# briangodwinlim/SIR-GCN

Measured on AMD Instinct MI355X. Metric: edges/sec SIRConv fwd+bwd, d_hidden=256, 1/2/4/8 MI355X, higher is better.
Workload: dtype f32; 1 GPU; cfg4 S2: Chung-Lu power-law V=2000000 E=40000000 alpha=0.8; 1 SIRConv layer d_in=H=d_out=256, agg=sum, LeakyReLU(0.2), f32, feat_dropout=0.0; fwd+bwd incl. projections; graph=S2, V=2000000, E=40000000, hidden=256, agg=sum, parallelism=single GPU

## Files before the change

### sir-gcn_amd/csrc/sirconv_gemm.hip

```cpp
#include <type_traits>
#include <algorithm>

#include "sirconv_internal.h"
#include "sirconv_gemm_util.h"
#include "sirconv_dropout.h"
#include "sirconv_gemm_nt.h"

namespace sir {
namespace {
using namespace gemm;

__device__ inline void kahan_add(float& s, float& c, float x) {
    const float y = x - c;
    const float t = s + y;
    c = (t - s) - y;
    s = t;
}

__device__ inline float gate_dact(float g, float x, int relu, float slope) {
    return g > 0.f ? x : (relu ? 0.f : x * slope);
}
__global__ void __launch_bounds__(256)
k_gate_dact_bits(float* __restrict__ C, int64_t ldc, const uint64_t* __restrict__ mask, int64_t M, int relu, float slope) {
    const int64_t i = (int64_t)blockIdx.x * 256 + threadIdx.x;
// ... 454 lines not shown
                }
            }
            __syncthreads();
#pragma unroll
            for (int i = 0; i < 8; ++i) {
                const int ir = wq + 8 * i, c16 = lq;
                u4v v = *reinterpret_cast<const u4v*>(img + ir * PITCH + c16 * 16);
                const int ml = (ir >> 5) * (TDT * 32) + 32 * b + (ir & 31);
                const int n = p.f0 + 4 * c16;
                const uint32_t off = (n < N) ? (uint32_t)ml * ldc4 + (uint32_t)c16 * 16u : nrec;
                if constexpr (GATE == 2) {
                    const u4v m01 = __builtin_amdgcn_raw_buffer_load_b128(grs, (uint32_t)ml * 32u, 0, 0);
                    const u4v m23 = __builtin_amdgcn_raw_buffer_load_b128(grs, (uint32_t)ml * 32u + 16u, 0, 0);
                    const int sh = c16 & 31;
                    const uint32_t w0 = c16 < 32 ? m01.x : m01.y, w1 = c16 < 32 ? m01.z : m01.w;
                    const uint32_t w2 = c16 < 32 ? m23.x : m23.y, w3 = c16 < 32 ? m23.z : m23.w;
                    const float g0 = ((w0 >> sh) & 1u) ? 1.f : -1.f, g1 = ((w1 >> sh) & 1u) ? 1.f : -1.f;
                    const float g2 = ((w2 >> sh) & 1u) ? 1.f : -1.f, g3 = ((w3 >> sh) & 1u) ? 1.f : -1.f;
                    v.x = __float_as_uint(gate_dact(g0, __uint_as_float(v.x), gate_relu, gate_slope));
                    v.y = __float_as_uint(gate_dact(g1, __uint_as_float(v.y), gate_relu, gate_slope));
                    v.z = __float_as_uint(gate_dact(g2, __uint_as_float(v.z), gate_relu, gate_slope));
                    v.w = __float_as_uint(gate_dact(g3, __uint_as_float(v.w), gate_relu, gate_slope));
                } else if constexpr (GATE == 1) {
                    const u4v gv = __builtin_amdgcn_raw_buffer_load_b128(grs, off, p.f0 * 4, 0);
                    v.x = __float_as_uint(gate_dact(__uint_as_float(gv.x), __uint_as_float(v.x), gate_relu, gate_slope));
                    v.y = __float_as_uint(gate_dact(__uint_as_float(gv.y), __uint_as_float(v.y), gate_relu, gate_slope));
                    v.z = __float_as_uint(gate_dact(__uint_as_float(gv.z), __uint_as_float(v.z), gate_relu, gate_slope));
                    v.w = __float_as_uint(gate_dact(__uint_as_float(gv.w), __uint_as_float(v.w), gate_relu, gate_slope));
                }
                __builtin_amdgcn_raw_buffer_store_b128(v, crs, off, p.f0 * 4, 0);
                __builtin_amdgcn_sched_barrier(0);
                asm volatile("s_nop 1" ::: "memory");
                __builtin_amdgcn_sched_barrier(0);
            }
            __syncthreads();
        }
    };

    TileP cur = tile_p(tb), nxt = tile_p(tb + 1);
    load_a(0, cur, 0);
    load_w(cur, 0);
    store(0, 0, true, false, 0);
    load_a(1, cur, 1);
    load_w(cur, 1);
    load_a(0, cur, 2);
    __syncthreads();
    typedef std::integral_constant<int, 0> I0;
    typedef std::integral_constant<int, 1> I1;
    typedef std::integral_constant<int, 2> I2;
    auto step = [&](int c, int j, const TileP& cu, const TileP& nx, auto P_, auto Z_, auto SK_, auto WN_, auto AN_) {
        constexpr int P = decltype(P_)::value, SK = decltype(SK_)::value;
        constexpr bool Z = decltype(Z_)::value != 0, WN = decltype(WN_)::value != 0, AN = decltype(AN_)::value != 0;
        if constexpr (!Z) rescale(P);
        mfma(P, Z);
        if constexpr (SK == 2) store(0, 0, true, false, 0);
        else store(P ^ 1, P ^ 1, false, SK == 1, j & 1);
        if constexpr (WN) load_w(nx, c + 2 - NCT);
        else load_w(cu, c + 2);
        if constexpr (AN) load_a(P ^ 1, nx, c + 3 - NCT);
        else load_a(P ^ 1, cu, c + 3);
        __syncthreads();
    };
    auto run = [&]() {
        TileP cu = cur, nx = nxt;
        for (int j = 0; tb + j < te; ++j) {
            const TileP nn = tile_p(tb + j + 2);
            step(0, j, cu, nx, I0(), I1(), I0(), I0(), I0());
#pragma unroll
            for (int c = 1; c + 1 <= NCT - 4; c += 2) {
                step(c, j, cu, nx, I1(), I0(), I0(), I0(), I0());
                step(c + 1, j, cu, nx, I0(), I0(), I0(), I0(), I0());
            }
            step(NCT - 3, j, cu, nx, I1(), I0(), I0(), I0(), I1());
            step(NCT - 2, j, cu, nx, I0(), I0(), I1(), I1(), I1());
            step(NCT - 1, j, cu, nx, I1(), I0(), I2(), I1(), I1());
            epilogue(cu, j & 1);
            cu = nx;
            nx = nn;
        }
    };
    run();
}

template <int WM, int WN, int TMT, int TNT>
__global__ void __launch_bounds__(64 * WM * WN)
k_gemm_tn(const float* __restrict__ A, int64_t lda, const float* __restrict__ B, int64_t ldb,
          int64_t R, int Mc, int Nc, float* __restrict__ part, float* __restrict__ csum_part,
          int n_mtiles, int n_ntiles, int64_t rows_per_split) {
    constexpr int NT = 64 * WM * WN;
    constexpr int BM = 32 * TMT * WM, BN = 32 * TNT * WN;
    constexpr int KSPT = 2 * (BM + BN) / NT;
    static_assert(KSPT * NT == 2 * (BM + BN) && (KSPT == 1 || KSPT == 2), "loader mapping");
    constexpr int XR = 16 * KSPT;
    constexpr int A_BYTES = BM * 128, B_BYTES = BN * 128;
    constexpr int STAGE = A_BYTES + B_BYTES + (BM + BN) * 4;
    __shared__ __attribute__((aligned(16))) char lds[2 * STAGE + 16];
    int* const rescaled = reinterpret_cast<int*>(lds + 2 * STAGE);

    const int t = threadIdx.x;
    const int wg = xcd_remap(blockIdx.x, gridDim.x);
    const int tiles = n_mtiles * n_ntiles;
    const int p = wg / tiles, tile = wg % tiles;
    const int m0 = (tile / n_ntiles) * BM, n0 = (tile % n_ntiles) * BN;
    const int64_t v_begin = (int64_t)p * rows_per_split;
    const int64_t v_end = (v_begin + rows_per_split < R) ? v_begin + rows_per_split : R;
    const int nc = (int)((v_end - v_begin + KC - 1) / KC);

    const int slot = KSPT == 1 ? (t >> 1) : t;
    const bool is_a = __builtin_amdgcn_readfirstlane(t >> 6) < BM * (2 / KSPT) / 64;
    const int cl = is_a ? slot : slot - BM, kse = KSPT == 1 ? (t & 1) : 0;
    const bool col_ok = is_a ? (m0 + cl < Mc) : (n0 + cl < Nc);
    const float* xbase = is_a ? A : B;
    const int ldx = (int)(is_a ? lda : ldb);
    const int xoff = 16 * kse * ldx + (is_a ? m0 : n0) + (col_ok ? cl : 0);
    const int img = is_a ? 0 : A_BYTES, rows_img = is_a ? BM : BN, fac_off = is_a ? cl : BM + cl;
    const int hi_off = img + kse * rows_img * 32 + fimg(cl, 0);
    const int lo_delta = 2 * rows_img * 32;
    const int fac_byte = A_BYTES + B_BYTES + fac_off * 4;
    int se_run = SE_INIT;

    const int w = t >> 6, l = t & 63, r = l & 31, h = l >> 5;
    const int m_w = (w / WN) * TMT * 32, n_w = (w % WN) * TNT * 32;

    float4 xv_[2][XR / 4];
    const bool do_cs = csum_part != nullptr && is_a;
    float cs = 0.f, csc = 0.f;
    auto load = [&](int set, int c) {
        float4 (&xv)[XR / 4] = xv_[set];
        const int64_t vc = v_begin + (int64_t)c * KC;
        const float* src = xbase + vc * ldx;
        float x[XR];
        const int64_t nrow = v_end - vc;
        const rsrc_t rs = mk_rsrc(src, nrow <= 0 ? 0u : (uint32_t)((nrow < KC ? nrow : KC) * ldx * 4));
#pragma unroll
        for (int j = 0; j < XR; ++j)
            x[j] = __uint_as_float(__builtin_amdgcn_raw_buffer_load_b32(rs, xoff * 4, j * ldx * 4, 0));
#pragma unroll
        for (int j = 0; j < XR / 4; ++j) xv[j] = make_float4(x[4 * j], x[4 * j + 1], x[4 * j + 2], x[4 * j + 3]);
    };
    auto store = [&](int set, int buf, int chunk, bool first = false) {
        const float4 (&xv)[XR / 4] = xv_[set];
        char* st = lds + buf * STAGE;
        float m = 0.f;
#pragma unroll
        for (int j = 0; j < XR / 4; ++j) m = fmax4_mix(m, xv[j]);
        if (KSPT == 1) m = fmaxf(m, __shfl_xor(m, 1));
        const int se_old = se_run, se = next_se(se_old, bexp(m));
        se_run = se;
        const float s = pow2(se);
#pragma unroll
        for (int q = 0; q < KSPT; ++q) {
            h8 hv[2], lv[2];
            split8_mix(xv[4 * q + 0], xv[4 * q + 1], s, hv[0], lv[0]);
            split8_mix(xv[4 * q + 2], xv[4 * q + 3], s, hv[1], lv[1]);
            char* hd = st + hi_off + q * rows_img * 32;
            *reinterpret_cast<h8*>(hd) = hv[0];
            *reinterpret_cast<h8*>(hd + 512) = hv[1];
            *reinterpret_cast<h8*>(hd + lo_delta) = lv[0];
            *reinterpret_cast<h8*>(hd + lo_delta + 512) = lv[1];
        }
        if (kse == 0) *reinterpret_cast<float*>(st + fac_byte) = first ? 1.f : pow2(se - se_old);
        if (do_cs) {
            float t = 0.f;
#pragma unroll
            for (int j = 0; j < XR / 4; ++j) { t += xv[j].x; t += xv[j].y; t += xv[j].z; t += xv[j].w; }
            kahan_add(cs, csc, t);
        }
        if (!first && se != se_old) rescaled[buf] = chunk;
    };

    f16v acc[TMT][TNT];
#pragma unroll
    for (int a = 0; a < TMT; ++a)
#pragma unroll
        for (int b = 0; b < TNT; ++b)
#pragma unroll
            for (int i = 0; i < 16; ++i) acc[a][b][i] = 0.f;

    auto compute = [&](int c) {
        const int buf = c & 1;
        const char* st = lds + buf * STAGE;
        if (rescaled[buf] == c) {
            const float* fac = reinterpret_cast<const float*>(st + A_BYTES + B_BYTES);
#pragma unroll
            for (int a = 0; a < TMT; ++a) {
                float fa[16];
#pragma unroll
                for (int g = 0; g < 4; ++g) {
                    const float4 f4 = *reinterpret_cast<const float4*>(fac + m_w + 32 * a + 8 * g + 4 * h);
                    fa[4 * g] = f4.x; fa[4 * g + 1] = f4.y; fa[4 * g + 2] = f4.z; fa[4 * g + 3] = f4.w;
                }
#pragma unroll
                for (int b = 0; b < TNT; ++b) {
                    const float fb = fac[BM + n_w + 32 * b + r];
#pragma unroll
                    for (int i = 0; i < 16; ++i) acc[a][b][i] *= fa[i] * fb;
                }
            }
        }
#pragma unroll
        for (int ks = 0; ks < 2; ++ks) {
            __builtin_amdgcn_sched_barrier(0);
            h8 af[TMT][2], bf[TNT][2];
#pragma unroll
            for (int pt = 0; pt < 2; ++pt) {
#pragma unroll
                for (int a = 0; a < TMT; ++a)
                    af[a][pt] = *reinterpret_cast<const h8*>(st + (pt * 2 + ks) * BM * 32 + fimg(m_w + 32 * a + r, h));
#pragma unroll
                for (int b = 0; b < TNT; ++b)
                    bf[b][pt] = *reinterpret_cast<const h8*>(st + A_BYTES + (pt * 2 + ks) * BN * 32 + fimg(n_w + 32 * b + r, h));
            }
#pragma unroll
            for (int a = 0; a < TMT; ++a)
#pragma unroll
                for (int b = 0; b < TNT; ++b)
                    acc[a][b] = __builtin_amdgcn_mfma_f32_32x32x16_f16(af[a][0], bf[b][0], acc[a][b], 0, 0, 0);
#pragma unroll
            for (int a = 0; a < TMT; ++a)
#pragma unroll
                for (int b = 0; b < TNT; ++b)
                    acc[a][b] = __builtin_amdgcn_mfma_f32_32x32x16_f16(af[a][0], bf[b][1], acc[a][b], 0, 0, 0);
#pragma unroll
            for (int a = 0; a < TMT; ++a)
#pragma unroll
                for (int b = 0; b < TNT; ++b)
                    acc[a][b] = __builtin_amdgcn_mfma_f32_32x32x16_f16(af[a][1], bf[b][0], acc[a][b], 0, 0, 0);
        }
    };

    if (t < 2) rescaled[t] = -1;
    if (nc > 0) {
        load(0, 0);
        load(1, 1);
        store(0, 0, 0, true);
    }
    __syncthreads();
    auto step = [&](int c, int set) {
        load(set, c + 2);
        compute(c);
        if (c + 1 < nc) store(set ^ 1, (c + 1) & 1, c + 1);
        __syncthreads();
    };
    int c = 0;
    for (; c + 2 <= nc; c += 2) {
        step(c, 0);
        step(c + 1, 1);
    }
    if (c < nc) step(c, 0);

    float* sc = reinterpret_cast<float*>(lds);
    if (kse == 0) sc[fac_off] = pow2(-se_run);
    __syncthreads();
    float* out = part + (int64_t)p * Mc * Nc;
#pragma unroll
    for (int b = 0; b < TNT; ++b) {
        const int nl = n_w + 32 * b + r;
        const int n = n0 + nl;
        const float ib = sc[BM + nl];
#pragma unroll
        for (int a = 0; a < TMT; ++a) {
#pragma unroll
            for (int i = 0; i < 16; ++i) {
                const int ml = m_w + 32 * a + (i & 3) + 8 * (i >> 2) + 4 * h;
                const int m = m0 + ml;
                if (m < Mc && n < Nc) out[(int64_t)m * Nc + n] = acc[a][b][i] * sc[ml] * ib;
            }
        }
    }
    if (do_cs && tile % n_ntiles == 0) {
        const float other = KSPT == 1 ? __shfl_xor(cs, 1) : 0.f;
        if (kse == 0 && col_ok) csum_part[(int64_t)p * Mc + m0 + cl] = KSPT == 1 ? cs + other : cs;
    }
}

__global__ void __launch_bounds__(256)
k_gemm_reduce(const float* __restrict__ part, int P, int64_t count, int Nc, float* __restrict__ C, int64_t ldc) {
    const int64_t i = (int64_t)blockIdx.x * 256 + threadIdx.x;
    if (i >= count) return;
    float s = 0.f;
    int q = 0;
    for (; q + 16 <= P; q += 16) {
        float v[16];
#pragma unroll
        for (int j = 0; j < 16; ++j) v[j] = part[(int64_t)(q + j) * count + i];
#pragma unroll
        for (int j = 0; j < 16; ++j) s += v[j];
    }
    for (; q < P; ++q) s += part[(int64_t)q * count + i];
    C[(i / Nc) * ldc + i % Nc] = s;
}

constexpr int S_FT = 2;

template <bool KFULL>
__global__ void __launch_bounds__(256)
k_gemm_nt_s(const float* __restrict__ A, int64_t lda, int64_t M, int K, const u4v* __restrict__ Wp, int Npad, int Kc,
            const float* __restrict__ inv_t, const float* __restrict__ bias, int N, float* __restrict__ C, int64_t ldc,
            int nfg, int64_t n_waves, Drop drop) {
    drop = drop_resolve(drop);
    const int l = threadIdx.x & 63, r = l & 31, h = l >> 5;
    const int64_t w = (int64_t)blockIdx.x * 4 + (threadIdx.x >> 6);
    if (w >= n_waves) return;
    const int64_t d0 = (w / nfg) * 32;
    const int f0 = (int)(w % nfg) * S_FT;
    const int rows = (M - d0 < 32) ? (int)(M - d0) : 32;
    const rsrc_t ars = mk_rsrc(A + d0 * lda, (uint32_t)(rows * lda * 4));
    const rsrc_t wrs = mk_rsrc(Wp, (uint32_t)((int64_t)Kc * 4 * Npad * 32));
    const int aoff = (r * (int)lda + 8 * h) * 4;
    const int woff = 16 * l;
    float4 av[2][4];
    u4v wv[2][S_FT][2][2];
    auto load = [&](int set, int c) {
#pragma unroll
        for (int i = 0; i < 4; ++i) {
            const u4v u = __builtin_amdgcn_raw_buffer_load_b128(ars, aoff + ((i >> 1) * 16 + (i & 1) * 4) * 4, c * KC * 4, 0);
            av[set][i] = make_float4(__uint_as_float(u.x), __uint_as_float(u.y), __uint_as_float(u.z), __uint_as_float(u.w));
        }
#pragma unroll
        for (int a = 0; a < S_FT; ++a)
#pragma unroll
            for (int pt = 0; pt < 2; ++pt)
#pragma unroll
                for (int ks = 0; ks < 2; ++ks)
                    wv[set][a][pt][ks] = __builtin_amdgcn_raw_buffer_load_b128(
                        wrs, woff, ((c * 2 + pt) * 2 + ks) * Npad * 32 + (f0 + a) * 1024, 0);
    };
    f16v acc[S_FT];
#pragma unroll
    for (int a = 0; a < S_FT; ++a)
#pragma unroll
        for (int i = 0; i < 16; ++i) acc[a][i] = 0.f;
// ... 469 lines not shown
    float pv[16];
    tile.result(pv, h);
    wait_vm<0>();
    __syncthreads();
    float* red = lds;
    float* cred = lds + G::RED;
    const int tile_id = w0 + W0 * w1;
    if (wk > 0) {
#pragma unroll
        for (int i = 0; i < 16; ++i) red[(((wk - 1) * W0 * W1 + tile_id) * 16 + i) * 64 + l] = pv[i];
    }
    if (do_cs) cred[(wk * G::L0 + w0 * 32 + j) * 2 + h] = tile.cs;
    __syncthreads();
    if (wk == 0) {
#pragma unroll
        for (int q = 1; q < WK; ++q) {
#pragma unroll
            for (int i = 0; i < 16; ++i) pv[i] += red[(((q - 1) * W0 * W1 + tile_id) * 16 + i) * 64 + l];
        }
        const int64_t r1 = a1 + 32 * w1 + j;
        if constexpr (EPI == 0) {
            if (r1 < n1lines) {
#pragma unroll
                for (int g = 0; g < 4; ++g) {
                    const int64_t n = a0 + 32 * w0 + 8 * g + 4 * h;
                    if (n < n0lines) {
                        float4 o = make_float4(pv[4 * g] + bb[g].x, pv[4 * g + 1] + bb[g].y, pv[4 * g + 2] + bb[g].z,
                                               pv[4 * g + 3] + bb[g].w);
                        if (drop.on()) drop4(drop, r1, (int)n, o);
                        *reinterpret_cast<float4*>(C + r1 * ldc + n) = o;
                    }
                }
            }
        } else {
            float* out = C + p * n0lines * n1lines;
            if (r1 < n1lines) {
#pragma unroll
                for (int i = 0; i < 16; ++i) {
                    const int64_t m = a0 + 32 * w0 + (i & 3) + 8 * (i >> 2) + 4 * h;
                    if (m < n0lines) out[m * n1lines + r1] = pv[i];
                }
            }
        }
    }
    SIR_LT_TRACE_AT(20, __builtin_amdgcn_s_memtime());
    SIR_LT_TRACE_AT(21, __builtin_amdgcn_s_memrealtime());
    if (do_cs && t < G::L0 && a0 + t < n0lines) {
        float sum = 0.f;
#pragma unroll
        for (int q = 0; q < WK; ++q) sum += cred[(q * G::L0 + t) * 2] + cred[(q * G::L0 + t) * 2 + 1];
        csum_part[p * n0lines + a0 + t] = sum;
    }
}

}

#ifndef SIR_SMALL_ROWS
#define SIR_SMALL_ROWS 16384
#endif
static int64_t gemm_small_rows() {
    const char* e = getenv("SIR_GEMM_SMALL_ROWS");
    return (e != nullptr && e[0] != 0) ? atoll(e) : (int64_t)SIR_SMALL_ROWS;
}

#ifndef SIR_TN_S_ROWS
#define SIR_TN_S_ROWS 512
#endif
#ifndef SIR_LT_NT
#define SIR_LT_NT -1
#endif
#ifndef SIR_LT_TN
#define SIR_LT_TN 2
#endif
static int lt_env(const char* name, int dflt) {
    const char* e = getenv(name);
    return (e != nullptr && e[0] != 0) ? atoi(e) : dflt;
}
#ifndef SIR_NT_2B
#define SIR_NT_2B -1
#endif
static bool nt_2b_auto(int K, int N) {
    return (K == 256 && (N == 256 || N == 512)) || (K == 512 && N == 256);
}
#ifndef SIR_LT_BLOCKS
#define SIR_LT_BLOCKS 512
#endif
static bool aligned16(const void* p, int64_t ld) { return ((uintptr_t)p & 15u) == 0 && ld % 4 == 0; }
static int gemm_tn_splits_lt(int64_t R, int64_t tiles, int KS, int64_t* rps) {
    int64_t P = (SIR_LT_BLOCKS + tiles - 1) / tiles;
    const int64_t pmax = (R + KS - 1) / KS;
    if (P > pmax) P = pmax;
    if (P > 32) P = 32;
    if (P < 1) P = 1;
    int64_t r = (R + P - 1) / P;
    r = (r + KS - 1) / KS * KS;
    *rps = r > 0 ? r : KS;
    P = (R + *rps - 1) / *rps;
    return (int)(P < 1 ? 1 : P);
}

static int gemm_tn_splits_s(int64_t R, int64_t, int64_t) {
    int64_t P = (R + SIR_TN_S_ROWS - 1) / SIR_TN_S_ROWS;
    if (P > 16) P = 16;
    if (P < 1) P = 1;
    return (int)P;
}

static hipError_t run_gemm_nt_s(const float* A, int64_t lda, int64_t M, int K, const void* packed, int N,
                                const float* bias, float* C, int64_t ldc, hipStream_t st, const Drop& drop) {
    const int np = (int)gemm_pack_npad(N), kc = (K + KC - 1) / KC;
    const u4v* wp = static_cast<const u4v*>(packed);
    const float* inv = reinterpret_cast<const float*>(static_cast<const char*>(packed) + (int64_t)kc * 4 * np * 32);
    const int nfg = (N + 32 * S_FT - 1) / (32 * S_FT);
    const int64_t waves = (M + 31) / 32 * nfg;
    const unsigned blocks = (unsigned)((waves + 3) / 4);
    if (K % KC == 0)
        hipLaunchKernelGGL(k_gemm_nt_s<true>, dim3(blocks), dim3(256), 0, st, A, lda, M, K, wp, np, kc, inv, bias, N, C,
                           ldc, nfg, waves, drop);
    else
        hipLaunchKernelGGL(k_gemm_nt_s<false>, dim3(blocks), dim3(256), 0, st, A, lda, M, K, wp, np, kc, inv, bias, N, C,
                           ldc, nfg, waves, drop);
    return hipGetLastError();
}

#ifndef SIR_LT_NS
#define SIR_LT_NS 3
#endif
struct NtW {
    const float* W;
    int64_t ldw;
    const float* W2;
    int64_t ldw2, split, bias_cols;
};
template <bool TRANS, int W0, int W1, int WK>
static void launch_nt_lt(const float* A, int64_t lda, int64_t M, int K, const NtW& w, int N, const float* bias,
                         float* C, int64_t ldc, hipStream_t st, const Drop& drop) {
    using G = Lt<!TRANS, true, W0, W1, WK, SIR_LT_NS>;
    const int nt0 = (N + G::L0 - 1) / G::L0;
    const int64_t nt1 = (M + G::L1 - 1) / G::L1;
    hipLaunchKernelGGL((k_gemm_lt<!TRANS, true, W0, W1, WK, SIR_LT_NS, 0>), dim3((unsigned)(nt0 * nt1)), dim3(G::NT), 0, st,
                       w.W, w.ldw, A, lda, (int64_t)N, M, (int64_t)K, nt0, (int)nt1, (int64_t)K, bias, C, ldc, nullptr,
                       drop, w.W2, w.ldw2, w.split, w.bias_cols);
}

static int nt_lt_auto(int64_t M, int N) {
    const int64_t ncu = device_cu_count();
    if ((int64_t)((N + 31) / 32) * ((M + 63) / 64) <= ncu) return 7;
    if ((int64_t)((N + 63) / 64) * ((M + 63) / 64) <= ncu) return 8;
    return 3;
}

hipError_t run_gemm_nt_direct(const float* A, int64_t lda, int64_t M, int K, const float* W, int64_t ldw, int trans,
                              int N, const float* bias, float* C, int64_t ldc, hipStream_t st, const Drop& drop,
                              const float* W2, int64_t ldw2, int64_t split, int64_t bias_cols) {
    if (M == 0 || N == 0) return hipSuccess;
    int lt = lt_env("SIR_LT_NT", SIR_LT_NT);
    if (lt < 0) lt = nt_lt_auto(M, N);
    const NtW w{W, ldw, W2, ldw2, W2 != nullptr ? split : INT64_MAX, bias_cols};
    if (lt > 0 && K % 4 == 0 && N % 4 == 0 && aligned16(A, lda) && aligned16(W, ldw) && ((uintptr_t)bias & 15u) == 0
        && (W2 == nullptr || aligned16(W2, ldw2)) && 128 * lda < ((int64_t)1 << 29)
        && (trans ? (int64_t)K * ldw : 128 * ldw) < ((int64_t)1 << 29)
        && (M + 31) / 32 * ((N + 31) / 32) < ((int64_t)1 << 31)) {
        switch (lt * 2 + (trans ? 1 : 0)) {
        case 2: launch_nt_lt<false, 2, 2, 1>(A, lda, M, K, w, N, bias, C, ldc, st, drop); break;
        case 3: launch_nt_lt<true, 2, 2, 1>(A, lda, M, K, w, N, bias, C, ldc, st, drop); break;
        case 4: launch_nt_lt<false, 1, 2, 2>(A, lda, M, K, w, N, bias, C, ldc, st, drop); break;
// ... 125 lines not shown

hipError_t run_gemm_reduce(const float* part, int P, int64_t count, int Nc, float* C, int64_t ldc, hipStream_t st) {
    if (count > 0)
        hipLaunchKernelGGL(k_gemm_reduce, dim3((unsigned)((count + 255) / 256)), dim3(256), 0, st, part, P, count, Nc, C,
                           ldc);
    return hipGetLastError();
}

#ifndef SIR_TN_MINROWS
#define SIR_TN_MINROWS 1024
#endif
int gemm_tn_splits(int64_t R, int64_t Mc, int64_t Nc) {
    const int64_t tiles = ((Mc + 255) / 256) * ((Nc + 255) / 256);
    int64_t P = (256 + tiles - 1) / tiles;
    const int64_t pmax = (R + SIR_TN_MINROWS - 1) / SIR_TN_MINROWS;
    if (P > pmax) P = pmax;
    if (P < 1) P = 1;
    return (int)P;
}

int64_t gemm_tn_workspace(int64_t R, int64_t Mc, int64_t Nc) {
    int64_t P = gemm_tn_splits(R, Mc, Nc);
    if (R < gemm_small_rows()) {
        const int64_t ps = gemm_tn_splits_s(R, Mc, Nc);
        if (ps > P) P = ps;
        if (P < 32) P = 32;
    }
    return P * (Mc * Nc + Mc) * 4;
}

static int lt_tn_w0(int lt) { return (lt == 1 || lt == 5) ? 2 : 1; }
static int lt_tn_w1(int lt) { return lt == 3 ? 1 : 2; }
static int lt_tn_ks(int lt) { return 32 * (lt == 1 ? 1 : (lt == 2 || lt == 5) ? 2 : 4); }
static int64_t lt_tn_tiles(int lt, int Mc, int Nc) {
    const int a = 32 * lt_tn_w0(lt), b = 32 * lt_tn_w1(lt);
    return (int64_t)((Mc + a - 1) / a) * ((Nc + b - 1) / b);
}
template <int W0, int W1, int WK>
static void launch_tn_lt(const float* A, int64_t lda, const float* B, int64_t ldb, int64_t R, int Mc, int Nc,
                         float* part, bool colsum, hipStream_t st) {
    using G = Lt<false, false, W0, W1, WK, SIR_LT_NS>;
    const int nt0 = (Mc + G::L0 - 1) / G::L0, nt1 = (Nc + G::L1 - 1) / G::L1;
    const int64_t tiles = (int64_t)nt0 * nt1;
    int64_t rl = 0;
    const int Pl = gemm_tn_splits_lt(R, tiles, G::KS, &rl);
    float* cp = colsum ? part + (int64_t)Pl * Mc * Nc : nullptr;
    hipLaunchKernelGGL((k_gemm_lt<false, false, W0, W1, WK, SIR_LT_NS, 1>), dim3((unsigned)(Pl * tiles)), dim3(G::NT), 0,
                       st, A, lda, B, ldb, (int64_t)Mc, (int64_t)Nc, R, nt0, nt1, rl, nullptr, part, (int64_t)0, cp,
                       Drop{});
}

hipError_t run_gemm_tn(const float* A, int64_t lda, const float* B, int64_t ldb, int64_t R, int Mc, int Nc,
                       float* C, int64_t ldc, float* colsum, void* workspace, hipStream_t st) {
    if (Mc == 0 || Nc == 0) return hipSuccess;
    const bool small = R < gemm_small_rows();
    const int P = small ? gemm_tn_splits_s(R, Mc, Nc) : gemm_tn_splits(R, Mc, Nc);
    const int64_t rps = (R + P - 1) / P;
    const int nmt = (Mc + 255) / 256, nnt = (Nc + 255) / 256;
    float* part = static_cast<float*>(workspace);
    float* cpart = colsum != nullptr ? part + (int64_t)P * Mc * Nc : nullptr;
    const int lt = lt_env("SIR_LT_TN", SIR_LT_TN);
    if (small && lt > 0 && lt <= 5 && aligned16(A, lda) && aligned16(B, ldb) && (Mc + 31) / 32 * ((Nc + 31) / 32) < (1 << 24)) {
        switch (lt) {
        case 1: launch_tn_lt<2, 2, 1>(A, lda, B, ldb, R, Mc, Nc, part, colsum != nullptr, st); break;
        case 2: launch_tn_lt<1, 2, 2>(A, lda, B, ldb, R, Mc, Nc, part, colsum != nullptr, st); break;
        case 3: launch_tn_lt<1, 1, 4>(A, lda, B, ldb, R, Mc, Nc, part, colsum != nullptr, st); break;
        case 4: launch_tn_lt<1, 2, 4>(A, lda, B, ldb, R, Mc, Nc, part, colsum != nullptr, st); break;
        default: launch_tn_lt<2, 2, 2>(A, lda, B, ldb, R, Mc, Nc, part, colsum != nullptr, st); break;
        }
        const int64_t tiles = lt_tn_tiles(lt, Mc, Nc);
        int64_t rl = 0;
        const int Pl = gemm_tn_splits_lt(R, tiles, lt_tn_ks(lt), &rl);
        float* cp = colsum != nullptr ? part + (int64_t)Pl * Mc * Nc : nullptr;
        const int64_t count = (int64_t)Mc * Nc;
        const int64_t nbm = (count + 255) / 256, nbc = colsum != nullptr ? (Mc + 255) / 256 : 0;
        hipLaunchKernelGGL(k_gemm_reduce2, dim3((unsigned)(nbm + nbc)), dim3(256), 0, st, part, Pl, count, Nc, C, ldc,
                           cp, Mc, colsum, nbm);
        return hipGetLastError();
    }
    if (small) {
        const int smt = (Mc + 31) / 32, snt = (Nc + 31) / 32;
        hipLaunchKernelGGL(k_gemm_tn_s, dim3((unsigned)((int64_t)P * smt * snt)), dim3(256), 0, st, A, lda, B, ldb, R,
                           Mc, Nc, part, cpart, smt, snt, rps);
    } else
    hipLaunchKernelGGL((k_gemm_tn<2, 4, 4, 2>), dim3((unsigned)(P * nmt * nnt)), dim3(512), 0, st,
                       A, lda, B, ldb, R, Mc, Nc, part, cpart, nmt, nnt, rps);
    const int64_t count = (int64_t)Mc * Nc;
    const int64_t nbm = (count + 255) / 256, nbc = colsum != nullptr ? (Mc + 255) / 256 : 0;
    hipLaunchKernelGGL(k_gemm_reduce2, dim3((unsigned)(nbm + nbc)), dim3(256), 0, st, part, P, count, Nc, C, ldc, cpart,
                       Mc, colsum, nbm);
    return hipGetLastError();
}

}
```

### sir-gcn_amd/csrc/sirconv_gemm16.hip

```cpp
#include "sirconv.h"
#include "sirconv_internal.h"
#include "sirconv_gemm_util.h"
#include "sirconv_dropout.h"

#include <type_traits>

namespace sir {
namespace {
using namespace gemm;

typedef _Float16 h8 __attribute__((ext_vector_type(8)));
typedef __bf16 b8 __attribute__((ext_vector_type(8)));
typedef float f16v __attribute__((ext_vector_type(16)));
typedef unsigned int u4v __attribute__((ext_vector_type(4)));

constexpr int KC16 = 32;
constexpr int NSET = 3;

template <bool BF>
__device__ inline f16v mfma16(u4v a, u4v b, f16v c) {
    if constexpr (BF)
        return __builtin_amdgcn_mfma_f32_32x32x16_bf16(__builtin_bit_cast(b8, a), __builtin_bit_cast(b8, b), c, 0, 0, 0);
    else
        return __builtin_amdgcn_mfma_f32_32x32x16_f16(__builtin_bit_cast(h8, a), __builtin_bit_cast(h8, b), c, 0, 0, 0);
}

template <bool BF, bool C32>
__device__ inline float rnd16(float x) {
    if constexpr (C32) return x;
    else if constexpr (BF) return (float)(__bf16)x;
    else return (float)(_Float16)x;
}

template <bool BF>
__device__ inline float widen(uint32_t bits16) {
    if constexpr (BF)
        return __uint_as_float(bits16 << 16);
    else
        return (float)__builtin_bit_cast(_Float16, (unsigned short)bits16);
}

template <bool BF, int BM = 256, int BN = 256, int WN = 4, int TMT = 4, int TNT = 2>
__global__ void __launch_bounds__(BM + BN)
k_gemm_tn16(const unsigned short* __restrict__ A, int64_t lda, const unsigned short* __restrict__ B, int64_t ldb,
            int64_t R, int Mc, int Nc, float* __restrict__ part, float* __restrict__ csum_part, int n_mtiles,
            int n_ntiles, int64_t rows_per_split) {
    constexpr int SLOTS = BM / 2 + BN / 2;
    constexpr int PLANE_A = BM * 32, PLANE_B = BN * 32;
    constexpr int A_BYTES = 2 * PLANE_A, B_BYTES = 2 * PLANE_B;
    constexpr int STAGE = A_BYTES + B_BYTES;
    static_assert((SLOTS & (SLOTS - 1)) == 0 && (BM / 2) % 64 == 0, "slot layout");
    static_assert((BM / (TMT * 32)) * (BN / (TNT * 32)) == (BM + BN) / 64 && BN / (TNT * 32) == WN, "wave tiling");
    __shared__ __attribute__((aligned(16))) char lds[2 * STAGE];

    const int t = threadIdx.x;
    const int wg = xcd_remap(blockIdx.x, gridDim.x);
    const int tiles = n_mtiles * n_ntiles;
    const int p = wg / tiles, tile = wg % tiles;
    const int m0 = (tile / n_ntiles) * BM, n0 = (tile % n_ntiles) * BN;
    const int64_t v_begin = (int64_t)p * rows_per_split;
    const int64_t v_end = (v_begin + rows_per_split < R) ? v_begin + rows_per_split : R;
    const int nc = v_end > v_begin ? (int)((v_end - v_begin + KC16 - 1) / KC16) : 0;

    const int slot = t & (SLOTS - 1), kse = t / SLOTS;
    const bool is_a = (__builtin_amdgcn_readfirstlane(t >> 6) % (SLOTS / 64)) < (BM / 2) / 64;
    const int pr = is_a ? slot : slot - BM / 2;
    const int c0 = 2 * pr;
    const bool col_ok = is_a ? (m0 + c0 < Mc) : (n0 + c0 < Nc);
    const unsigned short* xbase = is_a ? A : B;
    const int64_t ldx = is_a ? lda : ldb;
    const int voff = ((is_a ? m0 : n0) + (col_ok ? c0 : 0)) * 2 + kse * 16 * (int)ldx * 2;
    const int img = (is_a ? 0 : A_BYTES) + kse * (is_a ? PLANE_A : PLANE_B);

    const int w = t >> 6, l = t & 63, r = l & 31, h = l >> 5;
    const int m_w = (w / WN) * TMT * 32, n_w = (w % WN) * TNT * 32;

    const int rstride = (int)ldx * 2;
    uint32_t xs[NSET][16];
    auto load = [&](int set, int c) {
        const int64_t vc = v_begin + (int64_t)c * KC16;
        const int64_t nrow = v_end - vc;
        const rsrc_t rs = mk_rsrc(xbase + vc * ldx, nrow <= 0 ? 0u : (uint32_t)((nrow < KC16 ? nrow : KC16) * ldx * 2));
        int so = 0;
#pragma unroll
        for (int j = 0; j < 16; ++j) {
            xs[set][j] = __builtin_amdgcn_raw_buffer_load_b32(rs, voff, so, 0);
            so += rstride;
            asm volatile("" : "+s"(so));
        }
    };
    float cs0 = 0.f, cs1 = 0.f;
    const bool do_cs = csum_part != nullptr && is_a;
    auto store = [&](int set, int buf) {
        char* st = lds + buf * STAGE + img;
        u4v lo0, lo1, hi0, hi1;
        uint32_t* q[4] = {(uint32_t*)&lo0, (uint32_t*)&lo1, (uint32_t*)&hi0, (uint32_t*)&hi1};
#pragma unroll
        for (int i = 0; i < 4; ++i) {
            q[0][i] = __builtin_amdgcn_perm(xs[set][2 * i + 1], xs[set][2 * i], 0x05040100u);
            q[1][i] = __builtin_amdgcn_perm(xs[set][2 * i + 9], xs[set][2 * i + 8], 0x05040100u);
            q[2][i] = __builtin_amdgcn_perm(xs[set][2 * i + 1], xs[set][2 * i], 0x07060302u);
            q[3][i] = __builtin_amdgcn_perm(xs[set][2 * i + 9], xs[set][2 * i + 8], 0x07060302u);
        }
        *reinterpret_cast<u4v*>(st + fimg(c0, 0)) = lo0;
        *reinterpret_cast<u4v*>(st + fimg(c0, 1)) = lo1;
        *reinterpret_cast<u4v*>(st + fimg(c0 + 1, 0)) = hi0;
        *reinterpret_cast<u4v*>(st + fimg(c0 + 1, 1)) = hi1;
        if (do_cs) {
#pragma unroll
            for (int j = 0; j < 16; ++j) {
                cs0 += widen<BF>(xs[set][j] & 0xffffu);
                cs1 += widen<BF>(xs[set][j] >> 16);
            }
        }
    };

    f16v acc[TMT][TNT];
#pragma unroll
    for (int a = 0; a < TMT; ++a)
#pragma unroll
        for (int b = 0; b < TNT; ++b)
#pragma unroll
            for (int i = 0; i < 16; ++i) acc[a][b][i] = 0.f;

    auto mfma = [&](int buf) {
        const char* st = lds + buf * STAGE;
#pragma unroll
        for (int ks = 0; ks < 2; ++ks) {
            u4v af[TMT], bf[TNT];
#pragma unroll
            for (int a = 0; a < TMT; ++a)
                af[a] = *reinterpret_cast<const u4v*>(st + ks * PLANE_A + fimg(m_w + 32 * a + r, h));
#pragma unroll
            for (int b = 0; b < TNT; ++b)
                bf[b] = *reinterpret_cast<const u4v*>(st + A_BYTES + ks * PLANE_B + fimg(n_w + 32 * b + r, h));
#pragma unroll
            for (int a = 0; a < TMT; ++a)
#pragma unroll
                for (int b = 0; b < TNT; ++b) acc[a][b] = mfma16<BF>(af[a], bf[b], acc[a][b]);
        }
    };

    auto step_full = [&](int c, int s) {
        load(s, c + 3);
        mfma(c & 1);
        store((s + 1) % NSET, (c + 1) & 1);
        __syncthreads();
    };
    auto step_tail = [&](int c, int s) {
        mfma(c & 1);
        if (c + 1 < nc) store((s + 1) % NSET, (c + 1) & 1);
        __syncthreads();
    };
    if (nc > 0) {
        load(0, 0);
        load(1, 1);
        load(2, 2);
        store(0, 0);
        __syncthreads();
        int c = 0;
        for (; c + 3 < nc; c += 3) {
            step_full(c, 0);
            step_full(c + 1, 1);
            step_full(c + 2, 2);
        }
        step_tail(c, 0);
        if (c + 1 < nc) step_tail(c + 1, 1);
        if (c + 2 < nc) step_tail(c + 2, 2);
    }

    float* out = part + (int64_t)p * Mc * Nc;
#pragma unroll
    for (int b = 0; b < TNT; ++b) {
        const int n = n0 + n_w + 32 * b + r;
#pragma unroll
        for (int a = 0; a < TMT; ++a) {
#pragma unroll
            for (int i = 0; i < 16; ++i) {
                const int m = m0 + m_w + 32 * a + (i & 3) + 8 * (i >> 2) + 4 * h;
                if (m < Mc && n < Nc) out[(int64_t)m * Nc + n] = acc[a][b][i];
            }
        }
    }
    if (csum_part != nullptr && tile % n_ntiles == 0) {
        float* cl = reinterpret_cast<float*>(lds);
        __syncthreads();
        if (is_a && kse == 1) { cl[c0] = cs0; cl[c0 + 1] = cs1; }
        __syncthreads();
        if (is_a && kse == 0) {
            if (m0 + c0 < Mc) csum_part[(int64_t)p * Mc + m0 + c0] = cs0 + cl[c0];
            if (m0 + c0 + 1 < Mc) csum_part[(int64_t)p * Mc + m0 + c0 + 1] = cs1 + cl[c0 + 1];
        }
    }
}


template <int I, int N_, typename F>
__device__ __forceinline__ void static_for(F&& f) {
    if constexpr (I < N_) {
        f(std::integral_constant<int, I>());
        static_for<I + 1, N_>(f);
    }
}

__device__ inline uint32_t pack2(float a, float b, bool bf) {
    if (bf) return (uint32_t)__builtin_bit_cast(unsigned short, (__bf16)a) |
                   ((uint32_t)__builtin_bit_cast(unsigned short, (__bf16)b) << 16);
    return (uint32_t)__builtin_bit_cast(unsigned short, (_Float16)a) |
           ((uint32_t)__builtin_bit_cast(unsigned short, (_Float16)b) << 16);
}

template <bool BF, bool A32, bool C32, int KC, int NC, int NS, int BFT = 256>
__global__ void __launch_bounds__(512)
k_gemm_nt16(const void* __restrict__ A, int64_t lda, int64_t M, const u4v* __restrict__ Wp, int Npad,
            const float* __restrict__ bias, int N, void* __restrict__ C, int64_t ldc, unsigned short* __restrict__ Acopy,
            int64_t ldac, int n_ftiles, int n_tiles, int tiles_per_block, Drop drop) {
    drop = drop_resolve(drop);
    constexpr int BD = 256, TFT = 2, WF = BFT / (TFT * 32), WD = 8 / WF, TDT = BD / (WD * 32);
    constexpr int KS = KC / 16;
    constexpr int PLANE = 256 * 32;
    constexpr int PLANE_W = BFT * 32;
    constexpr int STAGE = KS * (PLANE + PLANE_W);
    constexpr int EA = A32 ? 4 : 2;
    constexpr int AV = (KC / 2) * EA / 16;
    constexpr int WV = KS * PLANE_W / (16 * 512);
    constexpr int EC = C32 ? 4 : 2;
    static_assert(KC == 32 || KC == 64, "chunk");
    static_assert(BFT == 256 || BFT == 128, "feature tile");
    static_assert(WV >= 1, "weight loader");
    static_assert(NS >= 2 && NS <= NC && NC % NS == 0, "register sets: a tile's chunks map to sets the same way");
    constexpr int IMG_ROWS = 32 * WD;
    constexpr int EPITCH = BFT * EC + 16;
    constexpr int EPI_BYTES = IMG_ROWS * EPITCH;
    __shared__ __attribute__((aligned(16))) char lds[2 * STAGE + 512 * 4 + EPI_BYTES];
    float* const bias_l = reinterpret_cast<float*>(lds + 2 * STAGE);
    char* const epi = lds + 2 * STAGE + 512 * 4;

// ... 101 lines not shown
#pragma unroll
                for (int g = 0; g < 4; ++g) {
                    const int nl = f_wq + 32 * a + 8 * g + 4 * hq;
                    const float4 bb = *reinterpret_cast<const float4*>(bias_l + p.f0 + nl);
                    float o0 = acc[a][b][4 * g + 0] + bb.x, o1 = acc[a][b][4 * g + 1] + bb.y;
                    float o2 = acc[a][b][4 * g + 2] + bb.z, o3 = acc[a][b][4 * g + 3] + bb.w;
                    if (drop.on()) {
                        const uint32_t rh = drop_row_hash(drop, p.d0 + (wq / WF) * (TDT * 32) + 32 * b + rq);
                        const int cc = drop.col0 + p.f0 + nl;
                        o0 = drop_keep(drop, rh, cc + 0) ? rnd16<BF, C32>(o0) * drop.scale : 0.f;
                        o1 = drop_keep(drop, rh, cc + 1) ? rnd16<BF, C32>(o1) * drop.scale : 0.f;
                        o2 = drop_keep(drop, rh, cc + 2) ? rnd16<BF, C32>(o2) * drop.scale : 0.f;
                        o3 = drop_keep(drop, rh, cc + 3) ? rnd16<BF, C32>(o3) * drop.scale : 0.f;
                    }
                    char* d = wrow + (32 * a + 8 * g) * EC;
                    if constexpr (C32) {
                        *reinterpret_cast<float4*>(d) = make_float4(o0, o1, o2, o3);
                    } else {
                        typedef unsigned int u2v __attribute__((ext_vector_type(2)));
                        u2v ov;
                        ov.x = pack2(o0, o1, BF);
                        ov.y = pack2(o2, o3, BF);
                        *reinterpret_cast<u2v*>(d) = ov;
                    }
                }
            }
            __syncthreads();
            constexpr int PR = BFT * EC / 16;
#pragma unroll
            for (int i = 0; i < IMG_ROWS * PR / 512; ++i) {
                const int q = tq + 512 * i;
                const int ir = q / PR, c16 = q % PR;
                const u4v v = *reinterpret_cast<const u4v*>(epi + ir * EPITCH + c16 * 16);
                const int ml = (ir >> 5) * (TDT * 32) + 32 * b + (ir & 31);
                const int n = p.f0 + c16 * (16 / EC);
                const uint32_t off = (n < N) ? (uint32_t)ml * ldcb + (uint32_t)c16 * 16u : nrec;
                __builtin_amdgcn_raw_buffer_store_b128(v, crs, off, p.f0 * EC, 0);
                __builtin_amdgcn_sched_barrier(0);
                asm volatile("s_nop 1" ::: "memory");
                __builtin_amdgcn_sched_barrier(0);
            }
            __syncthreads();
        }
    };

    TileP cu = tile_p(tb), nx = tile_p(tb + 1);
    static_for<0, NS>([&](auto I_) { load(decltype(I_)::value, cu, decltype(I_)::value); });
    store(0, 0, cu, 0);
    __syncthreads();
    for (int j = 0; tb + j < te; ++j) {
        const TileP nn = tile_p(tb + j + 2);
        static_for<0, NC>([&](auto C_) {
            constexpr int c = decltype(C_)::value;
            constexpr int s = c % NS;
            if constexpr (c + NS < NC) load(s, cu, c + NS);
            else load(s, nx, c + NS - NC);
            mfma(c & 1, c == 0);
            if constexpr (c == NC - 1) epilogue(cu);
            if constexpr (c + 1 < NC) store((c + 1) % NS, (c + 1) & 1, cu, c + 1);
            else store(0, 0, nx, 0);
            __syncthreads();
        });
        cu = nx;
        nx = nn;
    }
}

__global__ void __launch_bounds__(64)
k_pack16(const float* __restrict__ W, int64_t ldw, int N, int K, int trans, int bf, int Npad, unsigned short* __restrict__ out) {
    const int n = blockIdx.x;
    for (int k = threadIdx.x; k < K; k += 64) {
        const float x = (n < N) ? (trans ? W[(int64_t)k * ldw + n] : W[(int64_t)n * ldw + k]) : 0.f;
        const unsigned short b = bf ? __builtin_bit_cast(unsigned short, (__bf16)x) : __builtin_bit_cast(unsigned short, (_Float16)x);
        const int P = k >> 4, j = k & 15;
        out[((int64_t)P * Npad * 32 + fimg(n, j >> 3)) / 2 + (j & 7)] = b;
    }
}

}

#ifndef SIR_TN16_NARROW
#define SIR_TN16_NARROW 1
#endif
static bool tn16_narrow(int Mc, int Nc) {
    const char* e = getenv("SIR_TN16_NARROW");
    const int on = (e != nullptr && e[0] != 0) ? atoi(e) : SIR_TN16_NARROW;
    return on && (Mc <= 128 || Nc <= 128);
}

hipError_t run_gemm_tn16(const void* A, int64_t lda, const void* B, int64_t ldb, int64_t R, int Mc, int Nc, int dtype,
                         float* C, int64_t ldc, float* colsum, void* workspace, hipStream_t st) {
    if (Mc == 0 || Nc == 0) return hipSuccess;
    const int P = gemm_tn_splits(R, Mc, Nc);
    const int64_t rps = (R + P - 1) / P;
    const int nmt = (Mc + 255) / 256, nnt = (Nc + 255) / 256;
    float* part = static_cast<float*>(workspace);
    float* cpart = colsum != nullptr ? part + (int64_t)P * Mc * Nc : nullptr;
    const auto* a = static_cast<const unsigned short*>(A);
    const auto* b = static_cast<const unsigned short*>(B);
    if (tn16_narrow(Mc, Nc)) {
        const int nm = (Mc + 127) / 128, nn = (Nc + 127) / 128;
        const dim3 grid((unsigned)(P * nm * nn));
        if (dtype == SIR_DTYPE_BF16)
            hipLaunchKernelGGL((k_gemm_tn16<true, 128, 128, 2, 2, 2>), grid, dim3(256), 0, st, a, lda, b, ldb, R, Mc, Nc,
                               part, cpart, nm, nn, rps);
        else
            hipLaunchKernelGGL((k_gemm_tn16<false, 128, 128, 2, 2, 2>), grid, dim3(256), 0, st, a, lda, b, ldb, R, Mc, Nc,
                               part, cpart, nm, nn, rps);
    } else {
        const dim3 grid((unsigned)(P * nmt * nnt));
        if (dtype == SIR_DTYPE_BF16)
            hipLaunchKernelGGL(k_gemm_tn16<true>, grid, dim3(512), 0, st, a, lda, b, ldb, R, Mc, Nc, part, cpart, nmt, nnt,
                               rps);
        else
            hipLaunchKernelGGL(k_gemm_tn16<false>, grid, dim3(512), 0, st, a, lda, b, ldb, R, Mc, Nc, part, cpart, nmt, nnt,
                               rps);
    }
    hipError_t e = hipGetLastError();
    if (e != hipSuccess) return e;
    e = run_gemm_reduce(part, P, (int64_t)Mc * Nc, Nc, C, ldc, st);
    if (e != hipSuccess || colsum == nullptr) return e;
    return run_gemm_reduce(cpart, P, (int64_t)Mc, Mc, colsum, 0, st);
}


namespace {
template <int DT>
__global__ void __launch_bounds__(256)
k_dropout_apply(void* __restrict__ X, int64_t ldx, int64_t M, int N, Drop drop) {
    drop = drop_resolve(drop);
    const int64_t m = blockIdx.y;
    const uint32_t rh = drop_row_hash(drop, m);
    for (int n = blockIdx.x * 256 + threadIdx.x; n < N; n += gridDim.x * 256) {
        const bool k = drop_keep(drop, rh, drop.col0 + n);
        if constexpr (DT == SIR_DTYPE_F32) {
            float* p = static_cast<float*>(X) + m * ldx + n;
            *p = k ? *p * drop.scale : 0.f;
        } else if constexpr (DT == SIR_DTYPE_BF16) {
            __bf16* p = static_cast<__bf16*>(X) + m * ldx + n;
            *p = k ? (__bf16)((float)*p * drop.scale) : (__bf16)0.f;
        } else {
            _Float16* p = static_cast<_Float16*>(X) + m * ldx + n;
            *p = k ? (_Float16)((float)*p * drop.scale) : (_Float16)0.f;
        }
    }
}
}

hipError_t run_dropout_apply(void* X, int64_t ldx, int64_t M, int N, int dtype, const Drop& drop, hipStream_t st) {
    if (M == 0 || N == 0 || !drop.on()) return hipSuccess;
    if (M > 2147483647) return hipErrorInvalidValue;
    const dim3 grid((unsigned)((N + 255) / 256 < 4 ? (N + 255) / 256 : 4), (unsigned)M);
    if (dtype == SIR_DTYPE_F32) hipLaunchKernelGGL(k_dropout_apply<SIR_DTYPE_F32>, grid, dim3(256), 0, st, X, ldx, M, N, drop);
    else if (dtype == SIR_DTYPE_BF16) hipLaunchKernelGGL(k_dropout_apply<SIR_DTYPE_BF16>, grid, dim3(256), 0, st, X, ldx, M, N, drop);
    else hipLaunchKernelGGL(k_dropout_apply<SIR_DTYPE_F16>, grid, dim3(256), 0, st, X, ldx, M, N, drop);
    return hipGetLastError();
}

int64_t gemm_pack16_bytes(int64_t N, int64_t K) { return (N + 255) / 256 * 256 * K * 2; }

hipError_t run_gemm_pack16(const float* W, int64_t ldw, int N, int K, int trans, int dtype, void* packed, hipStream_t st) {
    const int np = (N + 255) / 256 * 256;
    hipLaunchKernelGGL(k_pack16, dim3(np), dim3(64), 0, st, W, ldw, N, K, trans, dtype == SIR_DTYPE_BF16 ? 1 : 0, np,
                       static_cast<unsigned short*>(packed));
    return hipGetLastError();
}

#ifndef SIR_NT16_KC
#define SIR_NT16_KC 32
#endif
#ifndef SIR_NT16_NS
#define SIR_NT16_NS 2
#endif
#ifndef SIR_NT16_NS32
#define SIR_NT16_NS32 2
#endif

#ifndef SIR_NT16_NARROW
#define SIR_NT16_NARROW 1
#endif
template <bool BF, bool A32, bool C32, int BFT>
static hipError_t launch_nt16_w(const void* A, int64_t lda, int64_t M, int K, const void* packed, int N, const float* bias,
                                void* C, int64_t ldc, unsigned short* Acopy, int64_t ldac, hipStream_t st, const Drop& drop) {
    const int np = (N + 255) / 256 * 256, nft = (N + BFT - 1) / BFT;
    const int64_t ntiles = (M + 255) / 256 * nft;
    const int ncu = device_cu_count();
    const int tpb = (int)((ntiles + ncu - 1) / ncu);
    const int nblk = (int)((ntiles + tpb - 1) / tpb);
    const auto* wp = static_cast<const u4v*>(packed);
    constexpr int KC = (SIR_NT16_KC == 64 && !A32) ? 64 : 32;
    constexpr int NS = A32 ? SIR_NT16_NS32 : SIR_NT16_NS;
    const int nc = K / KC;
#define SIR_NT16_L(NCV, NSV)                                                                                   \
    hipLaunchKernelGGL((k_gemm_nt16<BF, A32, C32, KC, NCV, NSV, BFT>), dim3((unsigned)nblk), dim3(512), 0, st, A, lda, \
                       M, wp, np, bias, N, C, ldc, Acopy, ldac, nft, (int)ntiles, tpb, drop)
    if (nc == 256 / KC) SIR_NT16_L(256 / KC, (NS <= 256 / KC ? NS : 256 / KC));
// ... 39 lines not shown
```

Baseline: 1.982 billion edges/s.

## Stagger B-loader waves in TN weight-gradient GEMMs to spread LDS stores

Adds a STAG template variant to the f32 and 16-bit TN GEMM kernels. In it, the waves that load B store the next chunk to LDS before issuing the next global load and computing, while the A-loader waves keep the original order. The goal is to desynchronise the global-load and LDS-store phases across waves within a workgroup, so memory traffic and MFMA work overlap better. By default it is enabled only for Nc=256 with Mc=256 or 512. The B waves prefetch one extra chunk ahead, which adds register pressure and makes the pipeline more complex.

```diff
diff --git a/sir-gcn_amd/csrc/sirconv_gemm.hip b/sir-gcn_amd/csrc/sirconv_gemm.hip
--- a/sir-gcn_amd/csrc/sirconv_gemm.hip
+++ b/sir-gcn_amd/csrc/sirconv_gemm.hip
@@ -560,7 +560,7 @@
     run();
 }
 
-template <int WM, int WN, int TMT, int TNT>
+template <int WM, int WN, int TMT, int TNT, bool STAG = false>
 __global__ void __launch_bounds__(64 * WM * WN)
 k_gemm_tn(const float* __restrict__ A, int64_t lda, const float* __restrict__ B, int64_t ldb,
           int64_t R, int Mc, int Nc, float* __restrict__ part, float* __restrict__ csum_part,
@@ -603,7 +603,7 @@
     float4 xv_[2][XR / 4];
     const bool do_cs = csum_part != nullptr && is_a;
     float cs = 0.f, csc = 0.f;
-    auto load = [&](int set, int c) {
+    auto load = [&](int set, int c) __attribute__((always_inline)) {
         float4 (&xv)[XR / 4] = xv_[set];
         const int64_t vc = v_begin + (int64_t)c * KC;
         const float* src = xbase + vc * ldx;
@@ -616,7 +616,7 @@
 #pragma unroll
         for (int j = 0; j < XR / 4; ++j) xv[j] = make_float4(x[4 * j], x[4 * j + 1], x[4 * j + 2], x[4 * j + 3]);
     };
-    auto store = [&](int set, int buf, int chunk, bool first = false) {
+    auto store = [&](int set, int buf, int chunk, bool first = false) __attribute__((always_inline)) {
         const float4 (&xv)[XR / 4] = xv_[set];
         char* st = lds + buf * STAGE;
         float m = 0.f;
@@ -655,7 +655,7 @@
 #pragma unroll
             for (int i = 0; i < 16; ++i) acc[a][b][i] = 0.f;
 
-    auto compute = [&](int c) {
+    auto compute = [&](int c) __attribute__((always_inline)) {
         const int buf = c & 1;
         const char* st = lds + buf * STAGE;
         if (rescaled[buf] == c) {
@@ -708,24 +708,44 @@
     };
 
     if (t < 2) rescaled[t] = -1;
-    if (nc > 0) {
-        load(0, 0);
-        load(1, 1);
-        store(0, 0, 0, true);
-    }
-    __syncthreads();
-    auto step = [&](int c, int set) {
-        load(set, c + 2);
-        compute(c);
-        if (c + 1 < nc) store(set ^ 1, (c + 1) & 1, c + 1);
+    static_assert(!STAG || BM * (2 / KSPT) / 64 == WM * WN / 2, "the late half is the B loaders");
+    const bool late = STAG && !is_a;
+    auto run = [&](auto step) {
+        int c = 0;
+        for (; c + 2 <= nc; c += 2) {
+            step(c, 0);
+            step(c + 1, 1);
+        }
+        if (c < nc) step(c, 0);
+    };
+    if (late) {
+        if (nc > 0) {
+            load(0, 0);
+            load(1, 1);
+            store(0, 0, 0, true);
+            load(0, 2);
+        }
         __syncthreads();
-    };
-    int c = 0;
-    for (; c + 2 <= nc; c += 2) {
-        step(c, 0);
-        step(c + 1, 1);
-    }
-    if (c < nc) step(c, 0);
+        run([&](int c, int set) __attribute__((always_inline)) {
+            if (c + 1 < nc) store(set ^ 1, (c + 1) & 1, c + 1);
+            load(set ^ 1, c + 3);
+            compute(c);
+            __syncthreads();
+        });
+    } else {
+        if (nc > 0) {
+            load(0, 0);
+            load(1, 1);
+            store(0, 0, 0, true);
+        }
+        __syncthreads();
+        run([&](int c, int set) __attribute__((always_inline)) {
+            load(set, c + 2);
+            compute(c);
+            if (c + 1 < nc) store(set ^ 1, (c + 1) & 1, c + 1);
+            __syncthreads();
+        });
+    }
 
     float* sc = reinterpret_cast<float*>(lds);
     if (kse == 0) sc[fac_off] = pow2(-se_run);
@@ -1361,6 +1381,10 @@
 static bool nt_2b_auto(int K, int N) {
     return (K == 256 && (N == 256 || N == 512)) || (K == 512 && N == 256);
 }
+#ifndef SIR_TN_STAG
+#define SIR_TN_STAG -1
+#endif
+static bool tn_stag_auto(int Mc, int Nc) { return Nc == 256 && (Mc == 256 || Mc == 512); }
 #ifndef SIR_LT_BLOCKS
 #define SIR_LT_BLOCKS 512
 #endif
@@ -1652,9 +1676,15 @@
         const int smt = (Mc + 31) / 32, snt = (Nc + 31) / 32;
         hipLaunchKernelGGL(k_gemm_tn_s, dim3((unsigned)((int64_t)P * smt * snt)), dim3(256), 0, st, A, lda, B, ldb, R,
                            Mc, Nc, part, cpart, smt, snt, rps);
-    } else
-    hipLaunchKernelGGL((k_gemm_tn<2, 4, 4, 2>), dim3((unsigned)(P * nmt * nnt)), dim3(512), 0, st,
-                       A, lda, B, ldb, R, Mc, Nc, part, cpart, nmt, nnt, rps);
+    } else {
+        const int stag = lt_env("SIR_TN_STAG", SIR_TN_STAG);
+        if (stag < 0 ? tn_stag_auto(Mc, Nc) : stag != 0)
+            hipLaunchKernelGGL((k_gemm_tn<2, 4, 4, 2, true>), dim3((unsigned)(P * nmt * nnt)), dim3(512), 0, st,
+                               A, lda, B, ldb, R, Mc, Nc, part, cpart, nmt, nnt, rps);
+        else
+            hipLaunchKernelGGL((k_gemm_tn<2, 4, 4, 2, false>), dim3((unsigned)(P * nmt * nnt)), dim3(512), 0, st,
+                               A, lda, B, ldb, R, Mc, Nc, part, cpart, nmt, nnt, rps);
+    }
     const int64_t count = (int64_t)Mc * Nc;
     const int64_t nbm = (count + 255) / 256, nbc = colsum != nullptr ? (Mc + 255) / 256 : 0;
     hipLaunchKernelGGL(k_gemm_reduce2, dim3((unsigned)(nbm + nbc)), dim3(256), 0, st, part, P, count, Nc, C, ldc, cpart,
diff --git a/sir-gcn_amd/csrc/sirconv_gemm16.hip b/sir-gcn_amd/csrc/sirconv_gemm16.hip
--- a/sir-gcn_amd/csrc/sirconv_gemm16.hip
+++ b/sir-gcn_amd/csrc/sirconv_gemm16.hip
@@ -40,7 +40,7 @@
         return (float)__builtin_bit_cast(_Float16, (unsigned short)bits16);
 }
 
-template <bool BF, int BM = 256, int BN = 256, int WN = 4, int TMT = 4, int TNT = 2>
+template <bool BF, int BM = 256, int BN = 256, int WN = 4, int TMT = 4, int TNT = 2, bool STAG = false>
 __global__ void __launch_bounds__(BM + BN)
 k_gemm_tn16(const unsigned short* __restrict__ A, int64_t lda, const unsigned short* __restrict__ B, int64_t ldb,
             int64_t R, int Mc, int Nc, float* __restrict__ part, float* __restrict__ csum_part, int n_mtiles,
@@ -77,7 +77,7 @@
 
     const int rstride = (int)ldx * 2;
     uint32_t xs[NSET][16];
-    auto load = [&](int set, int c) {
+    auto load = [&](int set, int c) __attribute__((always_inline)) {
         const int64_t vc = v_begin + (int64_t)c * KC16;
         const int64_t nrow = v_end - vc;
         const rsrc_t rs = mk_rsrc(xbase + vc * ldx, nrow <= 0 ? 0u : (uint32_t)((nrow < KC16 ? nrow : KC16) * ldx * 2));
@@ -91,7 +91,7 @@
     };
     float cs0 = 0.f, cs1 = 0.f;
     const bool do_cs = csum_part != nullptr && is_a;
-    auto store = [&](int set, int buf) {
+    auto store = [&](int set, int buf) __attribute__((always_inline)) {
         char* st = lds + buf * STAGE + img;
         u4v lo0, lo1, hi0, hi1;
         uint32_t* q[4] = {(uint32_t*)&lo0, (uint32_t*)&lo1, (uint32_t*)&hi0, (uint32_t*)&hi1};
@@ -123,7 +123,7 @@
 #pragma unroll
             for (int i = 0; i < 16; ++i) acc[a][b][i] = 0.f;
 
-    auto mfma = [&](int buf) {
+    auto mfma = [&](int buf) __attribute__((always_inline)) {
         const char* st = lds + buf * STAGE;
 #pragma unroll
         for (int ks = 0; ks < 2; ++ks) {
@@ -141,18 +141,46 @@
         }
     };
 
-    auto step_full = [&](int c, int s) {
-        load(s, c + 3);
-        mfma(c & 1);
-        store((s + 1) % NSET, (c + 1) & 1);
+    const bool late = STAG && __builtin_amdgcn_readfirstlane(t >> 6) >= (BM + BN) / 128;
+    if (nc > 0 && late) {
+        load(0, 0);
+        load(1, 1);
+        load(2, 2);
+        store(0, 0);
+        load(0, 3);
         __syncthreads();
-    };
-    auto step_tail = [&](int c, int s) {
-        mfma(c & 1);
-        if (c + 1 < nc) store((s + 1) % NSET, (c + 1) & 1);
-        __syncthreads();
-    };
-    if (nc > 0) {
+        auto step_full = [&](int c, int s) __attribute__((always_inline)) {
+            store((s + 1) % NSET, (c + 1) & 1);
+            load((s + 1) % NSET, c + 4);
+            mfma(c & 1);
+            __syncthreads();
+        };
+        auto step_tail = [&](int c, int s) __attribute__((always_inline)) {
+            if (c + 1 < nc) store((s + 1) % NSET, (c + 1) & 1);
+            mfma(c & 1);
+            __syncthreads();
+        };
+        int c = 0;
+        for (; c + 3 < nc; c += 3) {
+            step_full(c, 0);
+            step_full(c + 1, 1);
+            step_full(c + 2, 2);
+        }
+        step_tail(c, 0);
+        if (c + 1 < nc) step_tail(c + 1, 1);
+        if (c + 2 < nc) step_tail(c + 2, 2);
+    } else if (nc > 0) {
+        auto step_full = [&](int c, int s) __attribute__((always_inline)) {
+            load(s, c + 3);
+            mfma(c & 1);
+            store((s + 1) % NSET, (c + 1) & 1);
+            __syncthreads();
+        };
+        auto step_tail = [&](int c, int s) __attribute__((always_inline)) {
+            mfma(c & 1);
+            if (c + 1 < nc) store((s + 1) % NSET, (c + 1) & 1);
+            __syncthreads();
+        };
         load(0, 0);
         load(1, 1);
         load(2, 2);
@@ -420,6 +448,14 @@
 #ifndef SIR_TN16_NARROW
 #define SIR_TN16_NARROW 1
 #endif
+#ifndef SIR_TN16_STAG
+#define SIR_TN16_STAG -1
+#endif
+static bool tn16_stag(int Mc, int Nc) {
+    const char* e = getenv("SIR_TN16_STAG");
+    const int v = (e != nullptr && e[0] != 0) ? atoi(e) : SIR_TN16_STAG;
+    return v < 0 ? (Nc == 256 && (Mc == 256 || Mc == 512)) : v != 0;
+}
 static bool tn16_narrow(int Mc, int Nc) {
     const char* e = getenv("SIR_TN16_NARROW");
     const int on = (e != nullptr && e[0] != 0) ? atoi(e) : SIR_TN16_NARROW;
@@ -447,9 +483,16 @@
                                part, cpart, nm, nn, rps);
     } else {
         const dim3 grid((unsigned)(P * nmt * nnt));
-        if (dtype == SIR_DTYPE_BF16)
+        const bool stag = tn16_stag(Mc, Nc);
+        if (dtype == SIR_DTYPE_BF16 && stag)
+            hipLaunchKernelGGL((k_gemm_tn16<true, 256, 256, 4, 4, 2, true>), grid, dim3(512), 0, st, a, lda, b, ldb, R, Mc, Nc,
+                               part, cpart, nmt, nnt, rps);
+        else if (dtype == SIR_DTYPE_BF16)
             hipLaunchKernelGGL(k_gemm_tn16<true>, grid, dim3(512), 0, st, a, lda, b, ldb, R, Mc, Nc, part, cpart, nmt, nnt,
                                rps);
+        else if (stag)
+            hipLaunchKernelGGL((k_gemm_tn16<false, 256, 256, 4, 4, 2, true>), grid, dim3(512), 0, st, a, lda, b, ldb, R, Mc, Nc,
+                               part, cpart, nmt, nnt, rps);
         else
             hipLaunchKernelGGL(k_gemm_tn16<false>, grid, dim3(512), 0, st, a, lda, b, ldb, R, Mc, Nc, part, cpart, nmt, nnt,
                                rps);
```

Measured after the change: 1.997 billion edges/s, median of 5. Within noise of the previous version (+0.7%).
